# Graph-Machine-Learning-Group/sgp

Hardware: AMD Instinct MI355X
Metric: encoded node-steps/sec (higher is better)
Workload: dtype f32 (hop products: operands as fp16 hi + lo pairs, three 16-bit MFMA terms per product, fp32 accumulation -- agrees with fp32 to ~1e-7 of the operand scale; reservoir: recurrent products: state (|h| <= 1, x 2^14) and W_hh (per-row power-of-two scale) as two fp16 pieces (22 bits), hi*hi + hi*lo + lo*

## Files before the change

include/sgp_amd.h:

```cpp
#ifndef SGP_AMD_H
#define SGP_AMD_H

#include <stdint.h>

#ifdef __cplusplus
extern "C" {
#endif

#define SGP_ABI_VERSION 3

#define SGP_EINVAL   (-1)
#define SGP_EUNSUP   (-2)

#define SGP_ACT_TANH      0
#define SGP_ACT_RELU      1
#define SGP_ACT_SELF_NORM 2
#define SGP_ACT_IDENTITY  3
#define SGP_ACT_TANH_REL  4

typedef void* sgp_stream_t;

int sgp_abi_version(void);
const char* sgp_last_error(void);
const char* sgp_build_arch(void);
// ... 20 lines not shown
                       const int32_t* pred, int32_t run_if, sgp_stream_t stream);
int sgp_spmm_res_f32(const int32_t* uptr, const int32_t* ucol, const int32_t* usplit,
                     const int32_t* gptr, const int32_t* gsup, const int32_t* gidx, const float* gw,
                     const int32_t* rowmap,
                     int32_t n_tiles, int32_t max_union, int32_t max_tile_quads,
                     const float* X, int64_t x_row_stride, int64_t x_batch_stride,
                     const float* X_halo, int64_t xh_row_stride, int64_t xh_batch_stride,
                     int32_t n_own,
                     float* Y, int64_t y_row_stride, int64_t y_batch_stride,
                     int32_t n_rows, int32_t n_cols, int32_t batch, int32_t feat,
                     const int32_t* pred, int32_t run_if, sgp_stream_t stream);
int32_t sgp_spmm_res_max_union(void);
int32_t sgp_spmm_res_max_quads(void);
int sgp_spmm_res_tune(int32_t cfg);

int sgp_spmm_mix_f32(const int32_t* uptr, const int32_t* ucol, const int32_t* usplit,
                     const int32_t* gptr, const int32_t* gsup, const int32_t* gidx, const float* gw,
                     const int32_t* rowmap,
                     const int32_t* dptr, const int32_t* didx, const float* dw,
                     int32_t n_tiles, int32_t max_union, int32_t max_dense,
                     const float* X, int64_t x_row_stride, int64_t x_batch_stride,
                     const float* X_halo, int64_t xh_row_stride, int64_t xh_batch_stride,
                     int32_t n_own,
                     float* Y, int64_t y_row_stride, int64_t y_batch_stride,
                     int32_t n_rows, int32_t n_cols, int32_t batch, int32_t feat,
                     const int32_t* pred, int32_t run_if, sgp_stream_t stream);
int32_t sgp_spmm_mix_max_union(void);
int32_t sgp_spmm_mix_max_dense(int32_t halo);

int sgp_abs_max_f32(const float* X, int64_t x_row_stride, int64_t x_batch_stride,
                    int32_t n_rows, int32_t batch, int32_t feat, float* out, sgp_stream_t stream);


int sgp_col_stats_f32(const float* X, int64_t x_row_stride, int64_t x_batch_stride,
                      int32_t n_rows, int32_t batch, int32_t feat, int32_t t_stride, int32_t r_stride, int32_t accumulate,
                      float* stats, sgp_stream_t stream);

int sgp_split_prepare_f32(const float* stats, double n_samples, double s_eff, int32_t full,
                          const float* bound_in, float bound_scalar, float norm_inf, int32_t feat,
                          float* x_tab, float* bound_out, int32_t* flag, sgp_stream_t stream);

int sgp_spmm_split_f32(const int32_t* hdr, const int32_t* rowid, const int32_t* ucol, const void* afr,
                       const int32_t* adr, const float* rinv, int32_t n_tiles,
                       const float* X, int64_t x_row_stride, int64_t x_batch_stride,
                       const float* X_halo, int64_t xh_row_stride, int64_t xh_batch_stride, int32_t n_own,
                       float* Y, int64_t y_row_stride, int64_t y_batch_stride,
                       int32_t n_rows, int32_t n_cols, int32_t batch, int32_t feat,
                       const float* x_tab, int32_t accumulate, int32_t t_chunk, const int32_t* pred, int32_t run_if, sgp_stream_t stream);
int32_t sgp_spmm_split_chunks(void);
int32_t sgp_spmm_split_max_union(void);
int32_t sgp_spmm_split_waves(void);
int32_t sgp_spmm_split_rows_per_wave(void);
int32_t sgp_spmm_split_max_feat(void);

int sgp_spmm_split_wide_f32(const int32_t* hdr, const int32_t* rowid, const int32_t* ucol, const void* afr,
                            const int32_t* adr, const float* rinv, int32_t n_tiles,
                            const float* X, int64_t x_row_stride, int64_t x_batch_stride,
                            const float* X_halo, int64_t xh_row_stride, int64_t xh_batch_stride, int32_t n_own,
                            float* Y, int64_t y_row_stride, int64_t y_batch_stride,
                            int32_t n_rows, int32_t n_cols, int32_t batch, int32_t feat,
                            const float* x_tab, int32_t accumulate, int32_t t_chunk, const int32_t* pred, int32_t run_if, sgp_stream_t stream);
int32_t sgp_spmm_split_wide_chunks(void);
int32_t sgp_spmm_split_wide_max_union(void);
int32_t sgp_spmm_split_wide_waves(void);
int32_t sgp_spmm_split_wide_rows_per_wave(void);
int32_t sgp_spmm_split_wide_max_feat(void);

int64_t sgp_split_plan_deal(const int64_t* rowptr, const int64_t* col, int64_t n_rows, int64_t n_cols,
                            const int64_t* order, int64_t n_order,
                            int32_t waves, int32_t chunks, int32_t max_union, int32_t rows_per_wave,
                            int64_t* wave_of_row, int64_t* slot_of_row, int64_t* tile_of_wave, int64_t* rows_of_wave);
int sgp_split_plan_fill(const int64_t* rowptr, const int64_t* col, const float* val, int64_t n_rows, int64_t n_cols,
                        const int64_t* wave_of_row, const int64_t* slot_of_row, const int64_t* tile_of_wave,
                        const int64_t* rows_of_wave, int64_t n_waves, int64_t n_tiles,
                        int32_t waves, int32_t chunks, int32_t max_union,
                        int32_t* hdr, int32_t* rowid, int32_t* ucol, void* afr, int32_t* adr, float* rinv,
                        double* stats, int32_t threads);

int sgp_spmm_colblock_f32(const int32_t* plan, const int32_t* segptr, const int32_t* wg_row0,
                          int32_t n_wg, int32_t n_blocks,
                          const float* X, int64_t x_row_stride, int64_t x_batch_stride,
                          const float* X_halo, int64_t xh_row_stride, int64_t xh_batch_stride, int32_t n_own,
                          float* Y, int64_t y_row_stride, int64_t y_batch_stride,
                          int32_t n_rows, int32_t n_cols, int32_t batch, int32_t feat,
                          const int32_t* pred, int32_t run_if, sgp_stream_t stream);
int32_t sgp_spmm_colblock_rows_cap(void);
int32_t sgp_spmm_colblock_round_pad(void);

int32_t sgp_spmm_tiled_max_union(int32_t feat);
int32_t sgp_spmm_tiled_max_tile_rows(void);
int32_t sgp_spmm_tiled_max_row_edges(void);

int64_t sgp_reservoir_workspace_bytes(int32_t F, int32_t R);
int sgp_reservoir_f32(const float* x, int64_t x_row_stride, int64_t x_step_stride,
                      const float* w_ih, const float* w_hh, const float* b,
                      double alpha, int32_t act,
                      float* out, int64_t out_row_stride, int64_t out_step_stride,
                      float* h_state, void* workspace,
                      int32_t T, int32_t N, int32_t F, int32_t R,
                      sgp_stream_t stream);

int sgp_reservoir_pieces_f32(const float* x, int64_t x_row_stride, int64_t x_step_stride,
                             const float* w_ih, const float* w_hh, const float* b,
                             double alpha, int32_t act,
                             float* out, int64_t out_row_stride, int64_t out_step_stride,
                             float* h_state, void* workspace,
// ... 175 lines not shown
```

sgp_amd/csrc/spmm_split.hip:

```cpp
#define SGP_SPLIT_NW 16
#define SGP_SPLIT_NCH 7
#define SGP_SPLIT_SMAX 768
#define SGP_SPLIT_CR 3
#define SGP_SPLIT_NAME(x) sgp_spmm_split_##x
#include "spmm_split_impl.h"
```

sgp_amd/csrc/spmm_split_impl.h:

```cpp
#include "common.h"
#include <stdlib.h>
#include <type_traits>

namespace {

typedef _Float16 h8 __attribute__((ext_vector_type(8)));
typedef short s4v __attribute__((ext_vector_type(4)));
using sgp::f32x4;

#ifndef SGP_SPLIT_NW
#define SGP_SPLIT_NW 16
#endif
constexpr int NW = SGP_SPLIT_NW;
static_assert(NW == 8 || NW == 12 || NW == 16, "8, 12 or 16 waves x 16 rows");
#ifndef SGP_SPLIT_NCH
#define SGP_SPLIT_NCH 7
#endif
constexpr int NCH = SGP_SPLIT_NCH;
#ifndef SGP_SPLIT_SMAX
#define SGP_SPLIT_SMAX 768
#endif
constexpr int SMAX = SGP_SPLIT_SMAX;
constexpr int NLD = (SMAX + 16 * NW - 1) / (16 * NW);
constexpr int BUF = SMAX * 64;
#ifndef SGP_SPLIT_VSTAGE
#define SGP_SPLIT_VSTAGE 0
#endif
constexpr bool VSTAGE = SGP_SPLIT_VSTAGE != 0;
constexpr int NBUF = VSTAGE ? 2 : 3;
constexpr int HDR = 64;
constexpr int MAXFEAT = 1024;
#ifndef SGP_SPLIT_CR
#define SGP_SPLIT_CR 3
#endif
constexpr int CR = SGP_SPLIT_CR;
static_assert(BUF < 65536 - 512, "packed 16-bit transpose-read addresses");
static_assert(VSTAGE ? (CR >= 1 && CR + NLD <= NCH) : (CR >= NLD - 1 && CR + NLD < NCH),
              "conversion sits between the staging requests and the last chunk");
static_assert(NLD <= 7 && NBUF * BUF + 2 * MAXFEAT * 4 <= 160 * 1024, "three buffers and the scale table in 160 KB");

#ifndef SGP_SPLIT_RING
#define SGP_SPLIT_RING 3
#endif
constexpr int RING = SGP_SPLIT_RING;
static_assert(RING >= 2 && RING <= 4, "one to three chunks of operands in flight");

constexpr int conv_ops(int c) {
    if (VSTAGE) return (c == CR - 1 ? 1 : 0) + (c >= CR && c < CR + NLD ? 2 : 0);
    return c == CR ? 2 : (c > CR && c < CR + NLD ? 3 : (c == CR + NLD ? 2 : 0));
}
#ifndef SGP_SPLIT_ACC3
#define SGP_SPLIT_ACC3 0
#endif
#ifndef SGP_SPLIT_SPREAD
#define SGP_SPLIT_SPREAD 0
#endif
constexpr bool SPREAD = SGP_SPLIT_SPREAD != 0;
constexpr int lgkm_behind(int c, bool conv) {
    int n = 4 * ((c + RING - 1 < NCH ? c + RING - 1 : NCH - 1) - c);
    if (SPREAD && c + RING - 1 < NCH) n -= 2;
    if (conv) for (int j = (c - (RING - 1) > 0 ? c - (RING - 1) : 0); j < c; ++j) n += conv_ops(j);
    return n;
}
constexpr int lgkm_wait(int c, bool conv) { return lgkm_behind(c, conv) < 15 ? lgkm_behind(c, conv) : 15; }
static_assert(RING == 4 || (lgkm_behind(NCH - 1, true) <= 15 && lgkm_behind(CR + 1, true) <= 15 && lgkm_behind(CR + 2, true) <= 15),
              "the standard ring's waits are exact");

template <int I, int N, class F> __device__ __forceinline__ void static_for(F&& f) {
    if constexpr (I < N) { f(std::integral_constant<int, I>{}); static_for<I + 1, N>(f); }
}

#ifdef SGP_ABLATION
#define ABL(bit) ((a.mode & (bit)) != 0)
#else
#define ABL(bit) false
#endif

struct SplitArgs {
    const int* hdr; const int* rowid; const int* ucol; const h8* afr; const int* adr; const float* rinv;
    int n_tiles, tiles_per_xcd;
    int time_major;
    const float* X; long long xrs, xbs;
    const float* XH; long long xhrs, xhbs;
    int n_own;
    float* Y; long long yrs, ybs;
    int batch, nslice, t_chunk;
    const float* xtab;
    const int* pred; int pred_want;
    unsigned long long* dbg;
    int mode;
};

struct BOp { s4v h0, h1, l0, l1; };
__device__ __forceinline__ void tr_issue(BOp& b, unsigned a0, unsigned a1) {
    asm volatile("ds_read_b64_tr_b16 %0, %4\n\tds_read_b64_tr_b16 %1, %5\n\t"
                 "ds_read_b64_tr_b16 %2, %4 offset:256\n\tds_read_b64_tr_b16 %3, %5 offset:256"
                 : "=&v"(b.h0), "=&v"(b.h1), "=&v"(b.l0), "=&v"(b.l1) : "v"(a0), "v"(a1) : "memory");
}
__device__ __forceinline__ void tr_issue_hi(BOp& b, unsigned a0, unsigned a1) {
    asm volatile("ds_read_b64_tr_b16 %0, %2\n\tds_read_b64_tr_b16 %1, %3" : "=&v"(b.h0), "=&v"(b.h1) : "v"(a0), "v"(a1) : "memory");
}
__device__ __forceinline__ void tr_issue_lo(BOp& b, unsigned a0, unsigned a1) {
    asm volatile("ds_read_b64_tr_b16 %0, %2 offset:256\n\tds_read_b64_tr_b16 %1, %3 offset:256" : "=&v"(b.l0), "=&v"(b.l1) : "v"(a0), "v"(a1) : "memory");
}
template <int N> __device__ __forceinline__ void tr_wait(BOp& b) {
    asm volatile("s_waitcnt lgkmcnt(%4)" : "+v"(b.h0), "+v"(b.h1), "+v"(b.l0), "+v"(b.l1) : "n"(N));
}
__device__ __forceinline__ h8 cat8(s4v x, s4v y) {
    return __builtin_bit_cast(h8, __builtin_shufflevector(x, y, 0, 1, 2, 3, 4, 5, 6, 7));
}
__device__ __forceinline__ unsigned addr_lo(unsigned base, unsigned packed) {
    unsigned r;
    asm("v_add_u32_sdwa %0, %1, %2 dst_sel:DWORD dst_unused:UNUSED_PAD src0_sel:DWORD src1_sel:WORD_0" : "=v"(r) : "v"(base), "v"(packed));
    return r;
}
__device__ __forceinline__ unsigned addr_hi(unsigned base, unsigned packed) {
    unsigned r;
    asm("v_add_u32_sdwa %0, %1, %2 dst_sel:DWORD dst_unused:UNUSED_PAD src0_sel:DWORD src1_sel:WORD_1" : "=v"(r) : "v"(base), "v"(packed));
    return r;
}

__device__ __forceinline__ void lds_read16(f32x4& v, unsigned addr) {
    asm volatile("ds_read_b128 %0, %1" : "=&v"(v) : "v"(addr) : "memory");
}
template <int OFF> __device__ __forceinline__ void lds_read16_off(f32x4& v, unsigned addr) {
    asm volatile("ds_read_b128 %0, %1 offset:%2" : "=&v"(v) : "v"(addr), "n"(OFF) : "memory");
}
template <int OFF> __device__ __forceinline__ void lds_write8(unsigned addr, uint2 d) {
    asm volatile("ds_write_b64 %0, %1 offset:%2" :: "v"(addr), "v"(d), "n"(OFF) : "memory");
}

__device__ __forceinline__ void dma16(unsigned voff, const void* sbase, unsigned lds_off) {
    asm volatile("s_mov_b32 m0, %2\n\ts_nop 0\n\tglobal_load_lds_dwordx4 %0, %1"
                 :: "v"(voff), "s"(sbase), "s"(lds_off) : "memory");
}
__device__ __forceinline__ void dma16_vaddr(const void* vaddr, unsigned lds_off) {
    asm volatile("s_mov_b32 m0, %1\n\ts_nop 0\n\tglobal_load_lds_dwordx4 %0, off" :: "v"(vaddr), "s"(lds_off) : "memory");
}

__device__ __forceinline__ void vload16(f32x4& d, unsigned voff, const void* sbase) {
    asm volatile("global_load_dwordx4 %0, %1, %2" : "=&v"(d) : "v"(voff), "s"(sbase) : "memory");
}
__device__ __forceinline__ void vload16_vaddr(f32x4& d, const void* vaddr) {
    asm volatile("global_load_dwordx4 %0, %1, off" : "=&v"(d) : "v"(vaddr) : "memory");
}

#ifndef SGP_SPLIT_STORE_MOD
#define SGP_SPLIT_STORE_MOD ""
#endif
template <int OFF> __device__ __forceinline__ void store16(const void* sbase, unsigned voff, f32x4 d) {
    asm volatile("global_store_dwordx4 %0, %1, %2 offset:%3 " SGP_SPLIT_STORE_MOD :: "v"(voff), "v"(d), "s"(sbase), "n"(OFF) : "memory");
}

template <int N> __device__ __forceinline__ void wait_vm() { asm volatile("s_waitcnt vmcnt(%0)" :: "n"(N) : "memory"); }
__device__ __forceinline__ void wait_vm_n(int n) {
    switch (n) {
        case 0: wait_vm<0>(); break; case 1: wait_vm<1>(); break; case 2: wait_vm<2>(); break;
        case 3: wait_vm<3>(); break; case 4: wait_vm<4>(); break; case 5: wait_vm<5>(); break;
        case 6: wait_vm<6>(); break; default: wait_vm<7>(); break;
    }
}

__device__ __forceinline__ void split4(const f32x4 v, const f32x4 s, uint2& hi, uint2& lo) {
    unsigned h01, h23, l01, l23;
    asm("v_fma_mixlo_f16 %0, %1, %2, 0" : "=v"(h01) : "v"(v[0]), "v"(s[0]));
    asm("v_fma_mixhi_f16 %0, %1, %2, 0" : "+v"(h01) : "v"(v[1]), "v"(s[1]));
    asm("v_fma_mixlo_f16 %0, %1, %2, 0" : "=v"(h23) : "v"(v[2]), "v"(s[2]));
    asm("v_fma_mixhi_f16 %0, %1, %2, 0" : "+v"(h23) : "v"(v[3]), "v"(s[3]));
    asm("v_fma_mixlo_f16 %0, %1, %2, -%3 op_sel_hi:[0,0,1]" : "=&v"(l01) : "v"(v[0]), "v"(s[0]), "v"(h01));
    asm("v_fma_mixhi_f16 %0, %1, %2, -%3 op_sel:[0,0,1] op_sel_hi:[0,0,1]" : "+v"(l01) : "v"(v[1]), "v"(s[1]), "v"(h01));
    asm("v_fma_mixlo_f16 %0, %1, %2, -%3 op_sel_hi:[0,0,1]" : "=&v"(l23) : "v"(v[2]), "v"(s[2]), "v"(h23));
    asm("v_fma_mixhi_f16 %0, %1, %2, -%3 op_sel:[0,0,1] op_sel_hi:[0,0,1]" : "+v"(l23) : "v"(v[3]), "v"(s[3]), "v"(h23));
    hi.x = h01; hi.y = h23; lo.x = l01; lo.y = l23;
}

template <bool HALO, bool ACC>
__global__ __launch_bounds__(NW * 64, NW / 4) void spmm_split(SplitArgs a) {
    extern __shared__ __attribute__((aligned(16))) char lds[];
    if (a.pred != nullptr && a.pred[0] != a.pred_want) return;

    const int xcd = blockIdx.x & 7, j = blockIdx.x >> 3;
    const int tile = a.time_major ? j % a.n_tiles : xcd * a.tiles_per_xcd + j % a.tiles_per_xcd;
    const int tchunk = a.time_major ? (j / a.n_tiles) * 8 + xcd : j / a.tiles_per_xcd;
    if (tile >= a.n_tiles) return;
    const int t_begin = tchunk * a.t_chunk;
    const int t_end = min(a.batch, t_begin + a.t_chunk);
    if (t_begin >= t_end) return;

    const int tid = threadIdx.x, lane = tid & 63;
    const int wave = __builtin_amdgcn_readfirstlane(tid >> 6);
    const int src_tile = ABL(16) ? xcd * a.tiles_per_xcd : tile;
    const int nU = __builtin_amdgcn_readfirstlane(a.hdr[(size_t)src_tile * HDR + 2 * NW]);
    const unsigned lds0 = (unsigned)(size_t)(__attribute__((address_space(3))) char*)lds;
    const int feat = a.nslice * 16;

    {
        float* tab = (float*)(lds + NBUF * BUF);
        for (int i = tid; i < 2 * feat; i += NW * 64) tab[i] = a.xtab[i];
    }
    h8 af[NCH][2];
    unsigned ad[NCH];
    {
        const h8* ap = a.afr + ((size_t)(tile * NW + wave) * NCH * 2) * 64 + lane;
        const int* dp = a.adr + ((size_t)(tile * NW + wave) * NCH) * 64 + lane;
#pragma unroll
        for (int c = 0; c < NCH; ++c) {
            af[c][0] = ap[(c * 2 + 0) * 64];
            af[c][1] = ap[(c * 2 + 1) * 64];
            ad[c] = (unsigned)dp[c * 64];
        }
    }
    unsigned xoff[NLD];
    const int* uc = a.ucol + (size_t)src_tile * SMAX;
    int nld = 0;
#pragma unroll
    for (int i = 0; i < NLD; ++i) {
        const int s = (i * NW + wave) * 16 + (lane >> 2);
        const int c = uc[s < nU ? s : 0];
        if (HALO && c >= a.n_own)
            xoff[i] = 0x80000000u | ((unsigned)(c - a.n_own) * (unsigned)a.xhrs * 4u + (unsigned)(lane & 3) * 16u);
        else
            xoff[i] = (unsigned)c * (unsigned)a.xrs * 4u + (unsigned)(lane & 3) * 16u;
        if ((i * NW + wave) * 16 < nU) nld = i + 1;
    }
    const int* rid = a.rowid + (size_t)(tile * NW + wave) * 16;
    const int row_a = rid[lane & 15];
    const float rinv = a.rinv[(size_t)(tile * NW + wave) * 16 + (lane & 15)];
    const unsigned yo = row_a < 0 ? ~0u : (unsigned)row_a * (unsigned)a.yrs * 4u + 16u * (unsigned)(lane >> 4);
    __builtin_amdgcn_s_waitcnt(0x0F70);
    const unsigned own = lds0 + wave * 1024 + lane * 16;
    const unsigned cv_off = lds0 + wave * 1024 + (lane >> 5) * 512 + ((lane >> 2) & 7) * 32 + (lane & 3) * 8;
    const unsigned tab_cv = lds0 + NBUF * BUF + (lane & 3) * 16;
    const unsigned tab_rs = lds0 + NBUF * BUF + feat * 4 + (lane >> 4) * 16;

    auto piece = [&](unsigned off, const float* xb, const float* xh, unsigned lds_off) {
        if constexpr (HALO) {
            const char* b = (off & 0x80000000u) ? (const char*)xh : (const char*)xb;
            dma16_vaddr(b + (off & 0x7fffffffu), lds_off);
        } else {
            dma16(off, xb, lds_off);
        }
    };
    auto issue_dma = [&](int t, int sl, int buf) {
// ... 29 lines not shown
        });
    };
    if constexpr (VSTAGE) {
        asm volatile("s_waitcnt lgkmcnt(0)\n\ts_barrier" ::: "memory");
        issue_loads(dt, dsl); advance(dt, dsl);
        f32x4 s4;
        lds_read16(s4, tab_cv);
        wait_vm<0>();
        static_for<0, NLD>([&](auto I) {
            constexpr int i = decltype(I)::value;
            asm volatile("s_waitcnt lgkmcnt(0)" : "+v"(s4), "+v"(ld[i]) :: "memory");
            uint2 hi, lo;
            split4(ld[i], s4, hi, lo);
            lds_write8<i * NW * 1024>(cv_off, hi); lds_write8<i * NW * 1024 + 256>(cv_off, lo);
        });
        if (n_units <= 1) { dt = t_begin; dsl = 0; }
        issue_loads(dt, dsl); advance(dt, dsl);
        if (n_units <= 2) { dt = t_begin; dsl = 0; }
        asm volatile("s_waitcnt lgkmcnt(0)\n\ts_barrier" ::: "memory");
    } else {
        issue_dma(dt, dsl, 0); advance(dt, dsl);
        if (n_units > 1) { issue_dma(dt, dsl, 1); advance(dt, dsl); wait_vm_n(nld); } else wait_vm<0>();
        asm volatile("s_waitcnt lgkmcnt(0)\n\ts_barrier" ::: "memory");
        {
            f32x4 v[NLD], s4;
            lds_read16(s4, tab_cv);
#pragma unroll
            for (int i = 0; i < NLD; ++i) lds_read16(v[i], own + i * (NW * 1024));
            asm volatile("s_waitcnt lgkmcnt(0)" : "+v"(s4), "+v"(v[0]), "+v"(v[NLD - 1]), "+v"(v[NLD / 2]));
            static_for<0, NLD>([&](auto I) {
                constexpr int i = decltype(I)::value;
                uint2 hi, lo;
                split4(v[i], s4, hi, lo);
                lds_write8<i * NW * 1024>(cv_off, hi); lds_write8<i * NW * 1024 + 256>(cv_off, lo);
            });
        }
        asm volatile("s_waitcnt lgkmcnt(0)\n\ts_barrier" ::: "memory");

    }

    int t = t_begin, sl = 0;
    unsigned cur = 0, nxt = BUF, nn = 2 * BUF;
    f32x4 h0 = {0, 0, 0, 0};
    auto stamp = [&](int u, int k) {
        if (ABL(256) && blockIdx.x == 0 && lane == 0 && u >= 16 && u < 24)
            a.dbg[((u - 16) * NW + wave) * 8 + k] = __builtin_amdgcn_s_memtime();
    };
    const float* xb2 = ABL(64) ? a.X : a.X + (long long)dt * a.xbs + dsl * 16;
    const float* xh2 = HALO ? a.XH + (long long)dt * a.xhbs + dsl * 16 : nullptr;
    const long long x_wrap = a.xbs - 16 * (a.nslice - 1), xh_wrap = a.xhbs - 16 * (a.nslice - 1);
    float* ys = a.Y + (long long)t * a.ybs;
    const long long y_wrap = a.ybs - 16 * (a.nslice - 1);
    int sl1 = a.nslice > 1 ? 1 : 0;
    for (int u = 0; u < n_units; ++u) {
        stamp(u, 0);
        const bool dma_now = u + 2 < n_units && !ABL(1);
        const unsigned base2 = lds0 + nn + wave * 1024;
        const unsigned cbo = lds0 + cur;

        f32x4 acc0 = {0, 0, 0, 0}, acc1 = {0, 0, 0, 0};
#if SGP_SPLIT_ACC3
        f32x4 acc2 = {0, 0, 0, 0};
#endif
        f32x4 v, s4;
        BOp b[RING];
        stamp(u, 1);
#pragma unroll
        for (int c = 0; c < RING - 1; ++c) tr_issue(b[c], addr_lo(cbo, ad[c]), addr_hi(cbo, ad[c]));
        static_for<0, NCH>([&](auto C) {
            constexpr int c = decltype(C)::value;
            BOp& x = b[c % RING];
            unsigned na0 = 0, na1 = 0;
            if constexpr (c + RING - 1 < NCH) {
                na0 = addr_lo(cbo, ad[c + RING - 1]); na1 = addr_hi(cbo, ad[c + RING - 1]);
                if constexpr (SPREAD) tr_issue_hi(b[(c + RING - 1) % RING], na0, na1);
                else tr_issue(b[(c + RING - 1) % RING], na0, na1);
            }
            if (ABL(8)) tr_wait<lgkm_wait(c, false)>(x); else tr_wait<lgkm_wait(c, true)>(x);
            if (!ABL(2)) {
                const h8 bh = cat8(x.h0, x.h1), bl = cat8(x.l0, x.l1);
                acc0 = __builtin_amdgcn_mfma_f32_16x16x32_f16(bh, af[c][0], acc0, 0, 0, 0);
                if constexpr (SPREAD && c + RING - 1 < NCH) tr_issue_lo(b[(c + RING - 1) % RING], na0, na1);
                acc1 = __builtin_amdgcn_mfma_f32_16x16x32_f16(bl, af[c][0], acc1, 0, 0, 0);
#if SGP_SPLIT_ACC3
                acc2 = __builtin_amdgcn_mfma_f32_16x16x32_f16(bh, af[c][1], acc2, 0, 0, 0);
#else
                acc1 = __builtin_amdgcn_mfma_f32_16x16x32_f16(bh, af[c][1], acc1, 0, 0, 0);
#endif
            } else if constexpr (SPREAD && c + RING - 1 < NCH) tr_issue_lo(b[(c + RING - 1) % RING], na0, na1);
            if constexpr (VSTAGE) {
                if constexpr (c == CR - 1) lds_read16(s4, tab_cv + sl1 * 64);
                if constexpr (c >= CR && c < CR + NLD) {
                    constexpr int i = c - CR;
                    wait_vm<NLD - 1>();
                    if constexpr (i == 0) asm volatile("s_waitcnt lgkmcnt(%2)" : "+v"(s4), "+v"(ld[i]) : "n"(c + RING - 1 < NCH ? 4 : 0) : "memory");
                    else asm volatile("" : "+v"(ld[i]) :: "memory");
                    uint2 hi, lo;
                    split4(ld[i], s4, hi, lo);
                    const unsigned w = cv_off + nxt;
                    lds_write8<i * NW * 1024>(w, hi); lds_write8<i * NW * 1024 + 256>(w, lo);
                    vpiece(ld[i], xoff[i], xb2, xh2);
                }
            } else {
            if constexpr (c < NLD) { if (dma_now && c < nld) piece(xoff[c], xb2, xh2, base2 + c * (NW * 1024)); }
            }
            if constexpr (!VSTAGE && c >= CR && c <= CR + NLD) {
                if (!ABL(8)) {
// ... 3 lines not shown
                        lds_read16(s4, tab_cv + sl1 * 64);
                    } else {
                        asm volatile("s_waitcnt lgkmcnt(%2)" : "+v"(s4), "+v"(v) : "n"(c + RING - 1 < NCH ? 4 : 0));
                        uint2 hi, lo;
                        split4(v, s4, hi, lo);
                        const unsigned w = cv_off + nxt;
                        lds_write8<(i - 1) * NW * 1024>(w, hi); lds_write8<(i - 1) * NW * 1024 + 256>(w, lo);
                    }
                    if constexpr (i < NLD) lds_read16_off<i * NW * 1024>(v, own + nxt);
                }
            }
        });
        stamp(u, 3);
        if (!ABL(4)) {
            f32x4 iv;
            lds_read16(iv, tab_rs + sl * 64);
            asm volatile("s_waitcnt lgkmcnt(0)" : "+v"(iv));
#if SGP_SPLIT_ACC3
            acc1 += acc2;
#endif
            const f32x4 r0 = (acc0 + acc1) * (iv * rinv);
            if (!(sl & 1) && sl + 1 < a.nslice && !ABL(32)) {
                h0 = r0;
            } else if (yo != ~0u) {
                if constexpr (ACC) {
                    char* yb = (char*)ys + yo;
                    if ((sl & 1) && !ABL(32)) { *(f32x4*)(yb - 64) += h0; *(f32x4*)yb += r0; }
                    else *(f32x4*)yb += r0;
                } else {
                    if ((sl & 1) && !ABL(32)) { store16<-64>(ys, yo, h0); store16<0>(ys, yo, r0); }
                    else store16<0>(ys, yo, r0);
                }
            }
        }
        stamp(u, 5);
        if (VSTAGE ? u + 3 < n_units : dma_now) {
            const bool wrap = ++dsl == a.nslice;
            if (wrap) dsl = 0;
            if (!ABL(64)) xb2 += wrap ? x_wrap : 16;
            if (HALO) xh2 += wrap ? xh_wrap : 16;
        }
        {
            const bool wrap = sl + 1 == a.nslice;
            ys += wrap ? y_wrap : 16;
            sl = sl1;
            sl1 = sl1 + 1 == a.nslice ? 0 : sl1 + 1;
            if (wrap) ++t;
        }
        if constexpr (VSTAGE) { const unsigned f = cur; cur = nxt; nxt = f; }
        else { const unsigned f = cur; cur = nxt; nxt = nn; nn = f; }
        asm volatile("s_waitcnt lgkmcnt(0)\n\ts_barrier" ::: "memory");
        stamp(u, 6);
    }
}

}

extern "C" int32_t SGP_SPLIT_NAME(chunks)(void) { return NCH; }
extern "C" int32_t SGP_SPLIT_NAME(max_union)(void) { return SMAX; }
extern "C" int32_t SGP_SPLIT_NAME(waves)(void) { return NW; }
extern "C" int32_t SGP_SPLIT_NAME(rows_per_wave)(void) { return 16; }
extern "C" int32_t SGP_SPLIT_NAME(max_feat)(void) { return MAXFEAT; }

extern "C" int SGP_SPLIT_NAME(f32)(const int32_t* hdr, const int32_t* rowid, const int32_t* ucol, const void* afr,
                                  const int32_t* adr, const float* rinv,
                                  int32_t n_tiles,
                                  const float* X, int64_t x_row_stride, int64_t x_batch_stride,
                                  const float* X_halo, int64_t xh_row_stride, int64_t xh_batch_stride, int32_t n_own,
                                  float* Y, int64_t y_row_stride, int64_t y_batch_stride,
                                  int32_t n_rows, int32_t n_cols, int32_t batch, int32_t feat,
                                  const float* x_tab, int32_t accumulate, int32_t t_chunk, const int32_t* pred, int32_t run_if, sgp_stream_t stream) {
    const sgp::Predicate pr{pred, run_if};
    SGP_REQUIRE(n_tiles >= 0 && batch >= 0 && n_rows >= 0 && n_cols >= 0, "spmm_split: negative size");
    if (n_tiles == 0 || batch == 0 || n_rows == 0) return 0;
    SGP_REQUIRE(hdr && rowid && ucol && afr && adr && rinv && X && Y && x_tab, "spmm_split: null pointer");
    SGP_REQUIRE(feat > 0 && feat % 16 == 0 && feat <= MAXFEAT, "spmm_split: feat = %d is not a multiple of 16 up to %d", feat, MAXFEAT);
    SGP_REQUIRE(sgp::aligned16(X) && x_row_stride % 4 == 0 && x_batch_stride % 4 == 0 &&
                sgp::aligned16(Y) && y_row_stride % 4 == 0 && y_batch_stride % 4 == 0,
                "spmm_split: X and Y rows must be 16-byte aligned");
    {
        const long long own = X_halo ? n_own : n_cols, far = X_halo ? n_cols - n_own : 0;
        SGP_REQUIRE(own >= 0 && far >= 0 && own * x_row_stride < (1ll << 29) && far * xh_row_stride < (1ll << 29) &&
                    (long long)n_rows * y_row_stride < (1ll << 30), "spmm_split: rows beyond 32-bit byte offsets");
        SGP_REQUIRE(!X_halo || (sgp::aligned16(X_halo) && xh_row_stride % 4 == 0 && xh_batch_stride % 4 == 0),
                    "spmm_split: halo rows must be 16-byte aligned");
    }
    SplitArgs a;
    a.hdr = hdr; a.rowid = rowid; a.ucol = ucol; a.afr = (const h8*)afr; a.adr = adr; a.rinv = rinv;
    a.n_tiles = n_tiles; a.tiles_per_xcd = (n_tiles + 7) / 8;
    a.X = X; a.xrs = x_row_stride; a.xbs = x_batch_stride;
    a.XH = X_halo; a.xhrs = xh_row_stride; a.xhbs = xh_batch_stride; a.n_own = X_halo ? n_own : 0x7fffffff;
    a.Y = Y; a.yrs = y_row_stride; a.ybs = y_batch_stride;
    a.batch = batch; a.nslice = feat / 16;
    a.xtab = x_tab; a.pred = pr.flag; a.pred_want = pr.want;
    const bool auto_tc = t_chunk <= 0;
    if (t_chunk <= 0) {
        int cus = 256, dev = 0;
        if (hipGetDevice(&dev) != hipSuccess || hipDeviceGetAttribute(&cus, hipDeviceAttributeMultiprocessorCount, dev) != hipSuccess || cus < 1)
            cus = 256;
        double best = 1e30;
        for (int tc = 64; tc >= 8; tc >>= 1) {
            if (tc > batch && tc > 8) continue;
            const double w = (double)n_tiles * ((batch + tc - 1) / tc) / cus;
            const double cost = (w <= 1.0 ? 1.0 / w : (double)(long long)(w + 0.999999) / w) * (1.0 + 1.6 / tc);
            if (cost < best - 1e-9) { best = cost; t_chunk = tc; }
        }
        if (t_chunk <= 0) t_chunk = 8;
    }
    static const long tm_tune = sgp::tune("split_time_major", -1);
    static const long tm_tc = sgp::tune("split_tc", 0);
    a.time_major = tm_tune >= 0 ? (int)(tm_tune != 0) : (int)((long long)n_cols * feat * 4 <= (4ll << 20) && n_tiles >= 8);
    if (a.time_major) {
        if (tm_tc > 0 && auto_tc) t_chunk = (int)tm_tc;
        else if (auto_tc && n_tiles <= 32 && t_chunk > 16) t_chunk = 16;
    }
    a.t_chunk = t_chunk;
#ifdef SGP_ABLATION
    static const int abl = (int)sgp::tune("split_abl", 0);
#else
    constexpr int abl = 0;
#endif
    a.mode = abl;
    a.dbg = nullptr;
    if (abl & 256) { if (hipMalloc(&a.dbg, 8 * NW * 8 * 8) != hipSuccess) return sgp::fail(SGP_EINVAL, "dbg alloc"); (void)hipMemset(a.dbg, 0, 8 * NW * 8 * 8); }
    const int n_tchunks = (batch + t_chunk - 1) / t_chunk;
    auto kern = X_halo ? (accumulate ? spmm_split<true, true> : spmm_split<true, false>)
                       : (accumulate ? spmm_split<false, true> : spmm_split<false, false>);
    const int lds_bytes = NBUF * BUF + 2 * feat * 4;
    hipError_t e = hipFuncSetAttribute((const void*)kern, hipFuncAttributeMaxDynamicSharedMemorySize, NBUF * BUF + 2 * MAXFEAT * 4);
    if (e != hipSuccess) return sgp::fail((int)e, "spmm_split: LDS attribute: %s", hipGetErrorString(e));
    const unsigned grid = a.time_major ? 8u * (unsigned)n_tiles * (unsigned)((n_tchunks + 7) / 8)
                                       : 8u * (unsigned)a.tiles_per_xcd * (unsigned)n_tchunks;
    hipLaunchKernelGGL(kern, dim3(grid), dim3(NW * 64), lds_bytes, (hipStream_t)stream, a);
    if (abl & 256) {
        unsigned long long h[8 * NW * 8];
        (void)hipDeviceSynchronize();
        (void)hipMemcpy(h, a.dbg, sizeof(h), hipMemcpyDeviceToHost);
        (void)hipFree(a.dbg);
        printf("spmm_split timeline (cycles since the unit's top; columns: top | chunk loop start | - | chunk loop done | - | stores | barrier)\n");
        for (int u = 0; u < 8; ++u) for (int w = 0; w < NW; ++w) {
            const unsigned long long* r = h + (u * NW + w) * 8;
            printf("  unit %d wave %d: top %llu |", u, w, r[0] - h[0]);
            for (int k = 1; k < 7; ++k) printf(" %6lld", (long long)(r[k] - r[0]));
            printf("\n");
        }
    }
    return sgp::check_launch("spmm_split");
}
```

sgp_amd/hip.py:

```python
import ctypes
import json
import os
import subprocess

import torch

_CSRC = os.path.join(os.path.dirname(os.path.abspath(__file__)), "csrc")
LIB_PATH = os.environ.get("SGP_AMD_LIB") or os.path.join(_CSRC, "libsgp_amd.so")

c_i32, c_i64, c_f32, c_f64, c_p = (ctypes.c_int32, ctypes.c_int64,
                                   ctypes.c_float, ctypes.c_double,
                                   ctypes.c_void_p)
c_u64 = ctypes.c_uint64

SIGNATURES = {
    "sgp_abi_version": (ctypes.c_int, []),
    "sgp_last_error": (ctypes.c_char_p, []),
    "sgp_build_arch": (ctypes.c_char_p, []),
    "sgp_tune_value": (c_i64, [ctypes.c_char_p, c_i64]),
    "sgp_spmm_csr_f32": (ctypes.c_int, [c_p, c_p, c_p,
                                        c_p, c_i64, c_i64,
                                        c_p, c_i64, c_i64, c_i32,
                                        c_p, c_i64, c_i64,
                                        c_i32, c_i32, c_i32, c_i32, c_p, c_i32, c_p]),
# ... 63 lines not shown
                                                c_p,
                                                c_p, c_p, c_p, c_p, c_i32,
                                                c_p, c_p, c_i64,
                                                c_p, c_i32,
                                                c_i32, c_i32, c_i32, c_i32, c_i32, c_p]),
    "sgp_gesn_workspace_bytes": (c_i64, [c_i32, c_i32, c_i32]),
    "sgp_gesn_tune": (ctypes.c_int, [c_i32]),
    "sgp_gesn_f32": (ctypes.c_int, [c_p, c_p, c_p, c_p, c_i64, c_i64, c_p, c_p, c_p, c_p, c_i32,
                                    c_p, c_i64, c_i64, c_p, c_p,
                                    c_i32, c_i32, c_i32, c_i32, c_i32, c_p]),
    "sgp_gemm_nt_f32": (ctypes.c_int, [c_p, c_i64, c_p, c_i64, c_p, c_p, c_i64,
                                       c_i32, c_i32, c_i32, c_p]),
    "sgp_gesn_update_f32": (ctypes.c_int, [c_p, c_p, c_p, c_p, c_p, c_p, c_f64, c_i32,
                                           c_p, c_p, c_i64, c_i32, c_i32, c_p]),
    "sgp_node_mean_bcast_f32": (ctypes.c_int, [c_p, c_i64, c_i64,
                                               c_p, c_i64, c_i64, c_p,
                                               c_i32, c_i32, c_i32, c_p]),
    "sgp_bcast_rows_f32": (ctypes.c_int, [c_p, c_f32, c_p, c_i64, c_i64,
                                          c_i32, c_i32, c_i32, c_p]),
    "sgp_copy_rows_f32": (ctypes.c_int, [c_p, c_i64, c_i64, c_p, c_i64, c_i64,
                                         c_i32, c_i32, c_i32, c_p]),
    "sgp_gather_rows_f32": (ctypes.c_int, [c_p, c_i64, c_i64, c_p, c_p, c_i32,
                                           c_p, c_i64, c_i64, c_i32, c_i32, c_p]),
    "sgp_grouped_linear_packed_floats": (c_i64, [c_i32, c_i32, c_i32]),
    "sgp_grouped_linear_pack_f32": (ctypes.c_int, [c_p, c_p, c_i32, c_i32, c_i32, c_p]),
    "sgp_grouped_linear_f32": (ctypes.c_int, [c_p, c_i64, c_i64, c_p, c_p, c_p, c_p, c_i32,
                                              c_p, c_i64, c_i32, c_i32, c_i32, c_i32, c_p]),
    "sgp_grouped_linear_fwd_f32": (ctypes.c_int, [c_p, c_i64, c_i64, c_p, c_p, c_p, c_p, c_i32,
                                                  c_p, c_i64, c_p, c_f64, c_u64,
                                                  c_i32, c_i32, c_i32, c_i32, c_p]),
    "sgp_grouped_linear_dact_f32": (ctypes.c_int, [c_p, c_i64, c_p, c_i32, c_f64, c_u64, c_p, c_i64, c_i32, c_p]),
    "sgp_grouped_linear_transpose_f32": (ctypes.c_int, [c_p, c_p, c_i32, c_i32, c_i32, c_p]),
    "sgp_grouped_linear_wgrad_f32": (ctypes.c_int, [c_p, c_i64, c_i64, c_p, c_p, c_p, c_p,
                                                    c_i32, c_i32, c_i32, c_i32, c_p]),
    "sgp_abs_max_f32": (ctypes.c_int, [c_p, c_i64, c_i64, c_i32, c_i32, c_i32, c_p, c_p]),
    "sgp_spmm_split_f32": (ctypes.c_int, [c_p, c_p, c_p, c_p, c_p, c_p, c_i32, c_p, c_i64, c_i64,
                                          c_p, c_i64, c_i64, c_i32, c_p, c_i64, c_i64,
                                          c_i32, c_i32, c_i32, c_i32, c_p, c_i32, c_i32, c_p, c_i32, c_p]),
    "sgp_col_stats_f32": (ctypes.c_int, [c_p, c_i64, c_i64, c_i32, c_i32, c_i32, c_i32, c_i32, c_i32, c_p, c_p]),
    "sgp_split_prepare_f32": (ctypes.c_int, [c_p, c_f64, c_f64, c_i32, c_p, c_f32, c_f32, c_i32, c_p, c_p, c_p, c_p]),
    "sgp_spmm_split_wide_f32": (ctypes.c_int, [c_p, c_p, c_p, c_p, c_p, c_p, c_i32, c_p, c_i64, c_i64,
                                               c_p, c_i64, c_i64, c_i32, c_p, c_i64, c_i64,
                                               c_i32, c_i32, c_i32, c_i32, c_p, c_i32, c_i32, c_p, c_i32, c_p]),
    "sgp_spmm_split_wide_chunks": (c_i32, []),
    "sgp_spmm_split_wide_max_union": (c_i32, []),
    "sgp_spmm_split_wide_waves": (c_i32, []),
    "sgp_spmm_split_wide_rows_per_wave": (c_i32, []),
    "sgp_spmm_split_wide_max_feat": (c_i32, []),
    "sgp_spmm_split_chunks": (c_i32, []),
    "sgp_spmm_split_max_union": (c_i32, []),
    "sgp_spmm_split_waves": (c_i32, []),
    "sgp_spmm_split_rows_per_wave": (c_i32, []),
    "sgp_spmm_split_max_feat": (c_i32, []),
    "sgp_split_plan_deal": (c_i64, [c_p, c_p, c_i64, c_i64, c_p, c_i64, c_i32, c_i32, c_i32, c_i32, c_p, c_p, c_p, c_p]),
    "sgp_split_plan_fill": (ctypes.c_int, [c_p, c_p, c_p, c_i64, c_i64, c_p, c_p, c_p, c_p, c_i64, c_i64,
                                           c_i32, c_i32, c_i32, c_p, c_p, c_p, c_p, c_p, c_p, c_p, c_i32]),
    "sgp_spmm_colblock_f32": (ctypes.c_int, [c_p, c_p, c_p, c_i32, c_i32, c_p, c_i64, c_i64,
                                             c_p, c_i64, c_i64, c_i32, c_p, c_i64, c_i64,
                                             c_i32, c_i32, c_i32, c_i32, c_p, c_i32, c_p]),
    "sgp_spmm_colblock_rows_cap": (c_i32, []),
    "sgp_spmm_colblock_round_pad": (c_i32, []),
    "sgp_ridge_workspace_bytes": (c_i64, [c_i32, c_i64, c_i32, c_i32]),
    "sgp_ridge_colmeans_f32": (ctypes.c_int, [c_p, c_i32, c_p, c_i64, c_i64, c_p, c_p, c_i64, c_p]),
    "sgp_ridge_gram_f32": (ctypes.c_int, [c_p, c_i32, c_p, c_i64, c_i64, c_p, c_i32, c_p, c_i64, c_p, c_i64, c_p]),
    "sgp_ridge_predict_score_f32": (ctypes.c_int, [c_p, c_i32, c_p, c_i64, c_i64, c_p, c_p, c_i32, c_i32,
                                                   c_p, c_p, c_i64, c_p, c_i64, c_i64,
                                                   c_p, c_i64, c_i64, c_i64, c_p, c_p, c_p, c_i64, c_p]),
    "sgp_dense_packed_floats": (c_i64, [c_i32, c_i32]),
    "sgp_dense_pack_f32": (ctypes.c_int, [c_p, c_i64, c_i32, c_i32, c_i32, c_p, c_p]),
    "sgp_dense_f32": (ctypes.c_int, [c_p, c_i64, c_p, c_i64, c_p, c_p, c_i32, c_i32, c_i32,
                                     c_i32, c_i32, c_i32, c_p, c_i64, c_p, c_i64, c_f64, c_u64, c_i64,
                                     c_p, c_i64, c_p, c_p, c_p]),
    "sgp_dense_wgrad_workspace_floats": (c_i64, [c_i64, c_i32, c_i32, c_i32]),
    "sgp_dense_wgrad_f32": (ctypes.c_int, [c_p, c_i64, c_p, c_i64, c_p, c_i64, c_i32, c_i32, c_i32,
                                           c_p, c_i64, c_p, c_p, c_i64, c_p]),
    "sgp_row_segsum_f32": (ctypes.c_int, [c_p, c_i64, c_i64, c_i32, c_p, c_p, c_i32, c_p, c_p]),
    "sgp_masked_mae_f32": (ctypes.c_int, [c_p, c_p, c_p, c_i64, c_i32, c_p, c_p, c_p]),
    "sgp_masked_mae_bwd_f32": (ctypes.c_int, [c_p, c_p, c_p, c_i64, c_i32, c_p, c_p, c_p, c_p]),
    "sgp_gated_gn_supported": (c_i32, [c_i32, c_i32]),
    "sgp_gated_gn_chunk_edges": (c_i32, []),
    "sgp_gated_gn_workspace_bytes": (c_i64, [c_i32, c_i64, c_i64, c_i64, c_i32, c_i32]),
    "sgp_gated_gn_edge_f32": (ctypes.c_int, [c_p, c_i64, c_i32, c_i32, c_i32, c_i32, c_p, c_i32, c_p, c_i64,
                                             c_p, c_i32, c_i32, c_p, c_p, c_p, c_p, c_p, c_i64, c_p, c_i64, c_p]),
    "sgp_gated_gn_edge_bwd_f32": (ctypes.c_int, [c_p, c_i64, c_p, c_i64, c_i32, c_i32, c_i32, c_i32,
                                                 c_p, c_i32, c_p, c_i64, c_p, c_i32, c_i32, c_p, c_p,
                                                 c_p, c_p, c_p, c_p, c_p, c_p, c_i64, c_p, c_p, c_p, c_p,
                                                 c_p, c_i64, c_p]),
    "sgp_event_create": (ctypes.c_int, [ctypes.POINTER(c_p)]),
    "sgp_event_destroy": (ctypes.c_int, [c_p]),
    "sgp_event_record": (ctypes.c_int, [c_p, c_p]),
    "sgp_event_elapsed_ms": (ctypes.c_int, [c_p, c_p, ctypes.POINTER(c_f32)]),
}

ACT_CODES = {"tanh": 0, "relu": 1, "self_norm": 2, "identity": 3,
             "tanh_rel": 4}

_lib = None


def build(jobs=8, verbose=False, asan=False):
    out = subprocess.run(["make", "-C", _CSRC, f"-j{jobs}"], capture_output=True, text=True)
    if asan and out.returncode == 0:
        out = subprocess.run(["make", "-C", _CSRC, "-f", "Makefile.asan", f"-j{jobs}"], capture_output=True, text=True)
    if verbose or out.returncode:
        print(out.stdout[-4000:])
        print(out.stderr[-4000:])
# ... 935 lines not shown
```

Baseline: 1.261 billion.

## Add persistent gang scheduling with per-XCD window alignment to split SpMM

Replaces the one-block-per-(tile, time chunk) grid with a persistent grid of one gang of blocks per XCD. Each block walks whole tiles first and then shares the leftover tiles' time windows across gang members, which balances the tail. Blocks loosely align on time windows through a per-XCD atomic counter with bounded polling, so gang members stream the same X rows together and share them in cache. The cost is atomic and sleep overhead, a full vmem drain after each run, and the risk of stalls or imbalance if the polling estimate is off.

```diff
diff --git a/include/sgp_amd.h b/include/sgp_amd.h
--- a/include/sgp_amd.h
+++ b/include/sgp_amd.h
@@ -96,6 +96,9 @@
 int32_t sgp_spmm_split_waves(void);
 int32_t sgp_spmm_split_rows_per_wave(void);
 int32_t sgp_spmm_split_max_feat(void);
+int32_t sgp_spmm_split_mapping(int32_t n_tiles, int32_t n_cols, int32_t batch, int32_t feat, int32_t t_chunk);
+int32_t sgp_spmm_split_gang_run(int32_t n_tiles, int32_t batch, int32_t window, int32_t gang, int32_t xcd, int32_t member,
+                                int32_t k, int32_t* run);
 
 int sgp_spmm_split_wide_f32(const int32_t* hdr, const int32_t* rowid, const int32_t* ucol, const void* afr,
                             const int32_t* adr, const float* rinv, int32_t n_tiles,
diff --git a/sgp_amd/csrc/spmm_split.hip b/sgp_amd/csrc/spmm_split.hip
--- a/sgp_amd/csrc/spmm_split.hip
+++ b/sgp_amd/csrc/spmm_split.hip
@@ -3,4 +3,5 @@
 #define SGP_SPLIT_SMAX 768
 #define SGP_SPLIT_CR 3
 #define SGP_SPLIT_NAME(x) sgp_spmm_split_##x
+#define SGP_SPLIT_EXPORT_WALK 1
 #include "spmm_split_impl.h"
diff --git a/sgp_amd/csrc/spmm_split_impl.h b/sgp_amd/csrc/spmm_split_impl.h
--- a/sgp_amd/csrc/spmm_split_impl.h
+++ b/sgp_amd/csrc/spmm_split_impl.h
@@ -39,6 +39,9 @@
               "conversion sits between the staging requests and the last chunk");
 static_assert(NLD <= 7 && NBUF * BUF + 2 * MAXFEAT * 4 <= 160 * 1024, "three buffers and the scale table in 160 KB");
 
+#ifndef SGP_SPLIT_GANG_DEFAULT
+#define SGP_SPLIT_GANG_DEFAULT 1
+#endif
 #ifndef SGP_SPLIT_RING
 #define SGP_SPLIT_RING 3
 #endif
@@ -80,6 +83,8 @@
     const int* hdr; const int* rowid; const int* ucol; const h8* afr; const int* adr; const float* rinv;
     int n_tiles, tiles_per_xcd;
     int time_major;
+    int gang, gang_w, gang_polls;
+    unsigned* gang_cnt;
     const float* X; long long xrs, xbs;
     const float* XH; long long xhrs, xhbs;
     int n_own;
@@ -174,21 +179,58 @@
     hi.x = h01; hi.y = h23; lo.x = l01; lo.y = l23;
 }
 
-template <bool HALO, bool ACC>
-__global__ __launch_bounds__(NW * 64, NW / 4) void spmm_split(SplitArgs a) {
+struct GangShape {
+    int first, nf, r, nwin;
+    __host__ __device__ int pieces() const { return r * nwin; }
+    __host__ __device__ int windows(int G) const { return nf * nwin + (pieces() + G - 1) / G; }
+    __host__ __device__ int busiest(int G) const { const int m = pieces() % G; return m ? m : G; }
+};
+__host__ __device__ inline GangShape gang_shape(int n_tiles, int tiles_per_xcd, int T, int W, int G, int xcd) {
+    GangShape s;
+    s.first = xcd * tiles_per_xcd;
+    int ntx = n_tiles - s.first;
+    ntx = ntx < 0 ? 0 : (ntx > tiles_per_xcd ? tiles_per_xcd : ntx);
+    s.nf = ntx / G; s.r = ntx % G; s.nwin = (T + W - 1) / W;
+    return s;
+}
+__host__ __device__ inline bool gang_run(const GangShape& s, int T, int W, int G, int m, int k, int& tile, int& t0, int& t1) {
+    if (k < s.nf) { tile = s.first + k * G + m; t0 = 0; t1 = T; return true; }
+    if (k - s.nf > s.pieces() / G) return false;
+    const int i = (k - s.nf) * G + m;
+    if (i >= s.pieces()) return false;
+    tile = s.first + s.nf * G + i % s.r;
+    t0 = i / s.r * W;
+    t1 = t0 + W < T ? t0 + W : T;
+    return true;
+}
+__host__ __device__ inline unsigned gang_expected(const GangShape& s, int G, int j) {
+    const int n = s.windows(G);
+    return j <= n - 2 ? (unsigned)G * (unsigned)j : (unsigned)G * (unsigned)(n - 2) + (unsigned)s.busiest(G);
+}
+
+__device__ __forceinline__ void gang_align(const SplitArgs& a, const GangShape& gs, int xcd, int win) {
+    unsigned* cnt = a.gang_cnt + xcd * 8;
+    __hip_atomic_fetch_add(cnt, 1u, __ATOMIC_RELAXED, __HIP_MEMORY_SCOPE_AGENT);
+    const unsigned want = gang_expected(gs, a.gang, win);
+    for (int p = 0; p < a.gang_polls; ++p) {
+        if (__hip_atomic_load(cnt, __ATOMIC_RELAXED, __HIP_MEMORY_SCOPE_AGENT) >= want) break;
+        __builtin_amdgcn_s_sleep(8);
+    }
+}
+
+template <bool HALO, bool ACC, bool GANG>
+__device__ __forceinline__ void split_run(const SplitArgs& a, const int xcd, const int wave, const int tile, const int t_begin, const int t_end,
+                                          const GangShape& gs, int& gwin) {
     extern __shared__ __attribute__((aligned(16))) char lds[];
-    if (a.pred != nullptr && a.pred[0] != a.pred_want) return;
-
-    const int xcd = blockIdx.x & 7, j = blockIdx.x >> 3;
-    const int tile = a.time_major ? j % a.n_tiles : xcd * a.tiles_per_xcd + j % a.tiles_per_xcd;
-    const int tchunk = a.time_major ? (j / a.n_tiles) * 8 + xcd : j / a.tiles_per_xcd;
-    if (tile >= a.n_tiles) return;
-    const int t_begin = tchunk * a.t_chunk;
-    const int t_end = min(a.batch, t_begin + a.t_chunk);
-    if (t_begin >= t_end) return;
-
-    const int tid = threadIdx.x, lane = tid & 63;
-    const int wave = __builtin_amdgcn_readfirstlane(tid >> 6);
+    int lane, tid;
+    if constexpr (GANG) {
+        int zero = 0;
+        asm volatile("" : "+s"(zero));
+        lane = (int)__builtin_amdgcn_mbcnt_hi(~0u, __builtin_amdgcn_mbcnt_lo(~0u, (unsigned)zero));
+        tid = wave * 64 + lane;
+    } else {
+        tid = threadIdx.x; lane = tid & 63;
+    }
     const int src_tile = ABL(16) ? xcd * a.tiles_per_xcd : tile;
     const int nU = __builtin_amdgcn_readfirstlane(a.hdr[(size_t)src_tile * HDR + 2 * NW]);
     const unsigned lds0 = (unsigned)(size_t)(__attribute__((address_space(3))) char*)lds;
@@ -324,7 +366,17 @@
     float* ys = a.Y + (long long)t * a.ybs;
     const long long y_wrap = a.ybs - 16 * (a.nslice - 1);
     int sl1 = a.nslice > 1 ? 1 : 0;
+    int to_window = 0;
     for (int u = 0; u < n_units; ++u) {
+        if constexpr (GANG) {
+            if (to_window == 0) {
+                if (gwin > 0 && a.gang_cnt != nullptr && wave == 0 &&
+                    __builtin_amdgcn_mbcnt_hi(~0u, __builtin_amdgcn_mbcnt_lo(~0u, 0u)) == 0) gang_align(a, gs, xcd, gwin);
+                ++gwin;
+                to_window = a.gang_w * a.nslice;
+            }
+            --to_window;
+        }
         stamp(u, 0);
         const bool dma_now = u + 2 < n_units && !ABL(1);
         const unsigned base2 = lds0 + nn + wave * 1024;
@@ -434,6 +486,36 @@
         asm volatile("s_waitcnt lgkmcnt(0)\n\ts_barrier" ::: "memory");
         stamp(u, 6);
     }
+    if constexpr (GANG) wait_vm<0>();
+}
+
+template <bool HALO, bool ACC, bool GANG>
+__global__ __launch_bounds__(NW * 64, NW / 4) void spmm_split(SplitArgs a0) {
+    if (a0.pred != nullptr && a0.pred[0] != a0.pred_want) return;
+    const int xcd = blockIdx.x & 7, j = blockIdx.x >> 3;
+    const int wave = __builtin_amdgcn_readfirstlane(threadIdx.x >> 6);
+    if constexpr (!GANG) {
+        const SplitArgs& a = a0;
+        const int tile = a.time_major ? j % a.n_tiles : xcd * a.tiles_per_xcd + j % a.tiles_per_xcd;
+        const int tchunk = a.time_major ? (j / a.n_tiles) * 8 + xcd : j / a.tiles_per_xcd;
+        if (tile >= a.n_tiles) return;
+        const int t_begin = tchunk * a.t_chunk;
+        const int t_end = min(a.batch, t_begin + a.t_chunk);
+        if (t_begin >= t_end) return;
+        int gwin = 0;
+        split_run<HALO, ACC, false>(a, xcd, wave, tile, t_begin, t_end, GangShape{}, gwin);
+    } else {
+        const GangShape gs = gang_shape(a0.n_tiles, a0.tiles_per_xcd, a0.batch, a0.gang_w, a0.gang, xcd);
+        int gwin = 0;
+        for (int k = 0;; ++k) {
+            auto kargs = (const __attribute__((address_space(4))) SplitArgs*)__builtin_amdgcn_kernarg_segment_ptr();
+            asm volatile("" : "+s"(kargs));
+            const SplitArgs a = *(const SplitArgs*)kargs;
+            int tile, t_begin, t_end;
+            if (!gang_run(gs, a.batch, a.gang_w, a.gang, j, k, tile, t_begin, t_end)) break;
+            split_run<HALO, ACC, true>(a, xcd, wave, tile, t_begin, t_end, gs, gwin);
+        }
+    }
 }
 
 }
@@ -443,6 +525,63 @@
 extern "C" int32_t SGP_SPLIT_NAME(waves)(void) { return NW; }
 extern "C" int32_t SGP_SPLIT_NAME(rows_per_wave)(void) { return 16; }
 extern "C" int32_t SGP_SPLIT_NAME(max_feat)(void) { return MAXFEAT; }
+
+struct Mapping { int t_chunk, time_major, gang, gang_w, gang_polls; };
+static Mapping pick_mapping(int n_tiles, int n_cols, int batch, int feat, int t_chunk) {
+    Mapping mp{};
+    int cus = 256, dev = 0;
+    if (hipGetDevice(&dev) != hipSuccess || hipDeviceGetAttribute(&cus, hipDeviceAttributeMultiprocessorCount, dev) != hipSuccess || cus < 1)
+        cus = 256;
+    const bool auto_tc = t_chunk <= 0;
+    if (t_chunk <= 0) {
+        double best = 1e30;
+        for (int tc = 64; tc >= 8; tc >>= 1) {
+            if (tc > batch && tc > 8) continue;
+            const double w = (double)n_tiles * ((batch + tc - 1) / tc) / cus;
+            const double cost = (w <= 1.0 ? 1.0 / w : (double)(long long)(w + 0.999999) / w) * (1.0 + 1.6 / tc);
+            if (cost < best - 1e-9) { best = cost; t_chunk = tc; }
+        }
+        if (t_chunk <= 0) t_chunk = 8;
+    }
+    const long tm_tune = sgp::tune("split_time_major", -1);
+    const long tm_tc = sgp::tune("split_tc", 0);
+    mp.time_major = tm_tune >= 0 ? (int)(tm_tune != 0) : (int)((long long)n_cols * feat * 4 <= (4ll << 20) && n_tiles >= 8);
+    if (mp.time_major) {
+        if (tm_tc > 0 && auto_tc) t_chunk = (int)tm_tc;
+        else if (auto_tc && n_tiles <= 32 && t_chunk > 16) t_chunk = 16;
+    }
+    mp.t_chunk = t_chunk;
+    const long g_on = sgp::tune("split_gang", SGP_SPLIT_GANG_DEFAULT);
+    long g_size = sgp::tune("split_gang_size", 0);
+    const long g_w = sgp::tune("split_gang_w", 16), g_polls = sgp::tune("split_gang_polls", 64);
+    const int per_xcd = cus / 8 > 0 ? cus / 8 : 1;
+    if (g_size <= 0 || g_size > per_xcd) g_size = per_xcd;
+    if (g_on != 0 && !mp.time_major && auto_tc && (n_tiles + 7) / 8 >= g_size && g_w > 0 && g_w <= (1 << 20)) {
+        mp.gang = (int)g_size; mp.gang_w = (int)g_w;
+        mp.gang_polls = g_polls < -1 ? -1 : (g_polls > 4096 ? 4096 : (int)g_polls);
+    }
+    return mp;
+}
+
+#ifdef SGP_SPLIT_EXPORT_WALK
+extern "C" int32_t SGP_SPLIT_NAME(mapping)(int32_t n_tiles, int32_t n_cols, int32_t batch, int32_t feat, int32_t t_chunk) {
+    if (n_tiles <= 0 || n_cols <= 0 || batch <= 0 || feat <= 0) { sgp::fail(SGP_EINVAL, "spmm_split_mapping: sizes must be positive"); return -1; }
+    const Mapping mp = pick_mapping(n_tiles, n_cols, batch, feat, t_chunk);
+    return mp.gang > 0 ? 2 : mp.time_major;
+}
+extern "C" int32_t SGP_SPLIT_NAME(gang_run)(int32_t n_tiles, int32_t batch, int32_t window, int32_t gang, int32_t xcd, int32_t member,
+                                            int32_t k, int32_t* run) {
+    if (n_tiles <= 0 || batch <= 0 || window <= 0 || gang <= 0 || xcd < 0 || xcd >= 8 || member < 0 || member >= gang || k < 0 || !run) {
+        sgp::fail(SGP_EINVAL, "spmm_split_gang_run: bad argument");
+        return -1;
+    }
+    const GangShape gs = gang_shape(n_tiles, (n_tiles + 7) / 8, batch, window, gang, xcd);
+    int tile = 0, t0 = 0, t1 = 0;
+    if (!gang_run(gs, batch, window, gang, member, k, tile, t0, t1)) return 0;
+    run[0] = tile; run[1] = t0; run[2] = t1;
+    return 1;
+}
+#endif
 
 extern "C" int SGP_SPLIT_NAME(f32)(const int32_t* hdr, const int32_t* rowid, const int32_t* ucol, const void* afr,
                                   const int32_t* adr, const float* rinv,
@@ -475,27 +614,11 @@
     a.Y = Y; a.yrs = y_row_stride; a.ybs = y_batch_stride;
     a.batch = batch; a.nslice = feat / 16;
     a.xtab = x_tab; a.pred = pr.flag; a.pred_want = pr.want;
-    const bool auto_tc = t_chunk <= 0;
-    if (t_chunk <= 0) {
-        int cus = 256, dev = 0;
-        if (hipGetDevice(&dev) != hipSuccess || hipDeviceGetAttribute(&cus, hipDeviceAttributeMultiprocessorCount, dev) != hipSuccess || cus < 1)
-            cus = 256;
-        double best = 1e30;
-        for (int tc = 64; tc >= 8; tc >>= 1) {
-            if (tc > batch && tc > 8) continue;
-            const double w = (double)n_tiles * ((batch + tc - 1) / tc) / cus;
-            const double cost = (w <= 1.0 ? 1.0 / w : (double)(long long)(w + 0.999999) / w) * (1.0 + 1.6 / tc);
-            if (cost < best - 1e-9) { best = cost; t_chunk = tc; }
-        }
-        if (t_chunk <= 0) t_chunk = 8;
-    }
-    static const long tm_tune = sgp::tune("split_time_major", -1);
-    static const long tm_tc = sgp::tune("split_tc", 0);
-    a.time_major = tm_tune >= 0 ? (int)(tm_tune != 0) : (int)((long long)n_cols * feat * 4 <= (4ll << 20) && n_tiles >= 8);
-    if (a.time_major) {
-        if (tm_tc > 0 && auto_tc) t_chunk = (int)tm_tc;
-        else if (auto_tc && n_tiles <= 32 && t_chunk > 16) t_chunk = 16;
-    }
+    const Mapping mp = pick_mapping(n_tiles, n_cols, batch, feat, t_chunk);
+    t_chunk = mp.t_chunk;
+    a.time_major = mp.time_major;
+    a.gang = mp.gang; a.gang_w = mp.gang_w; a.gang_polls = mp.gang_polls;
+    a.gang_cnt = mp.gang > 0 && mp.gang_polls >= 0 ? sgp::sync_slot((hipStream_t)stream) : nullptr;
     a.t_chunk = t_chunk;
 #ifdef SGP_ABLATION
     static const int abl = (int)sgp::tune("split_abl", 0);
@@ -506,12 +629,15 @@
     a.dbg = nullptr;
     if (abl & 256) { if (hipMalloc(&a.dbg, 8 * NW * 8 * 8) != hipSuccess) return sgp::fail(SGP_EINVAL, "dbg alloc"); (void)hipMemset(a.dbg, 0, 8 * NW * 8 * 8); }
     const int n_tchunks = (batch + t_chunk - 1) / t_chunk;
-    auto kern = X_halo ? (accumulate ? spmm_split<true, true> : spmm_split<true, false>)
-                       : (accumulate ? spmm_split<false, true> : spmm_split<false, false>);
+    auto kern = a.gang > 0 ? (X_halo ? (accumulate ? spmm_split<true, true, true> : spmm_split<true, false, true>)
+                                     : (accumulate ? spmm_split<false, true, true> : spmm_split<false, false, true>))
+                           : (X_halo ? (accumulate ? spmm_split<true, true, false> : spmm_split<true, false, false>)
+                                     : (accumulate ? spmm_split<false, true, false> : spmm_split<false, false, false>));
     const int lds_bytes = NBUF * BUF + 2 * feat * 4;
     hipError_t e = hipFuncSetAttribute((const void*)kern, hipFuncAttributeMaxDynamicSharedMemorySize, NBUF * BUF + 2 * MAXFEAT * 4);
     if (e != hipSuccess) return sgp::fail((int)e, "spmm_split: LDS attribute: %s", hipGetErrorString(e));
-    const unsigned grid = a.time_major ? 8u * (unsigned)n_tiles * (unsigned)((n_tchunks + 7) / 8)
+    const unsigned grid = a.gang > 0 ? 8u * (unsigned)a.gang
+                        : a.time_major ? 8u * (unsigned)n_tiles * (unsigned)((n_tchunks + 7) / 8)
                                        : 8u * (unsigned)a.tiles_per_xcd * (unsigned)n_tchunks;
     hipLaunchKernelGGL(kern, dim3(grid), dim3(NW * 64), lds_bytes, (hipStream_t)stream, a);
     if (abl & 256) {
diff --git a/sgp_amd/hip.py b/sgp_amd/hip.py
--- a/sgp_amd/hip.py
+++ b/sgp_amd/hip.py
@@ -139,6 +139,8 @@
     "sgp_spmm_split_waves": (c_i32, []),
     "sgp_spmm_split_rows_per_wave": (c_i32, []),
     "sgp_spmm_split_max_feat": (c_i32, []),
+    "sgp_spmm_split_mapping": (c_i32, [c_i32, c_i32, c_i32, c_i32, c_i32]),
+    "sgp_spmm_split_gang_run": (c_i32, [c_i32, c_i32, c_i32, c_i32, c_i32, c_i32, c_i32, c_p]),
     "sgp_split_plan_deal": (c_i64, [c_p, c_p, c_i64, c_i64, c_p, c_i64, c_i32, c_i32, c_i32, c_i32, c_p, c_p, c_p, c_p]),
     "sgp_split_plan_fill": (ctypes.c_int, [c_p, c_p, c_p, c_i64, c_i64, c_p, c_p, c_p, c_p, c_i64, c_i64,
                                            c_i32, c_i32, c_i32, c_p, c_p, c_p, c_p, c_p, c_p, c_p, c_i32]),
```

New measurement: 1.248 billion. 1.1% lower.
